# QY-H00/attention-interpolation-diffusion

Hardware: AMD Instinct MI355X
Metric: interpolation-frames/sec (50-step) (higher is better)
Workload: dtype bf16

## Files before the change

attention-interpolation-diffusion_amd/csrc/aid_attn_pp.hip:

```cpp
#include <type_traits>

#include "aid_common.hpp"
#include "aid_kernels.hpp"

namespace aid {

namespace {

constexpr int PKT = 64;
constexpr int PTILE = 8192;
constexpr int PSTAGE = 2 * PTILE;
constexpr int PNS = 8;

struct AttnPPParams {
    AidAttnArgs a;
    int32_t nqb;
    int32_t multi;
    int32_t persist;
    int32_t hv_lo, hv_hi, hv_units;
    float   c2;
#ifdef AID_ABLATIONS
    int32_t abl;
#endif
};
// ... 16 lines not shown
    one[0] = (_Float16)1.0f; one[1] = (_Float16)1.0f;
    return __builtin_amdgcn_fdot2(__builtin_bit_cast(h2, w), one, acc, false);
}

template <typename V>
__device__ __forceinline__ V ld_uniform(const V* ptr, int i) {
    return reinterpret_cast<const __attribute__((address_space(4))) V*>(reinterpret_cast<uintptr_t>(ptr))[i];
}

#ifdef AID_ABLATIONS
#define PP_LDU(ptr, i) ((p.abl & 512) ? (ptr)[i] : ld_uniform(ptr, i))
#else
#define PP_LDU(ptr, i) ld_uniform(ptr, i)
#endif

template <int N>
__device__ __forceinline__ void wait_vm() {
    asm volatile("s_waitcnt vmcnt(%0)" ::"n"(N) : "memory");
}
__device__ __forceinline__ void slot_barrier() {
    __builtin_amdgcn_sched_barrier(0);
    __builtin_amdgcn_s_barrier();
    __builtin_amdgcn_sched_barrier(0);
}

template <typename T, int MODE>
__global__ __launch_bounds__(512) void aid_attn_pp_kernel(const AttnPPParams p) {
    typedef typename Vec<T>::v8 T8;
    typedef typename Vec<T>::v4 T4;
    constexpr int D = 64;
    constexpr float XTH = std::is_same<T, f16>::value ? 15.0f : 60.0f;
    constexpr bool SUMM = std::is_same<T, bf16>::value;
    constexpr float XB = SUMM ? XTH - 1.f : 0.f;
    typedef short s16x4 __attribute__((ext_vector_type(4)));
    extern __shared__ __attribute__((aligned(16))) char smem[];

#ifdef AID_ABLATIONS
    long long tl[6];
    tl[0] = clock64();
#endif
    const AidAttnArgs& a = p.a;
    const int tid = threadIdx.x, lane = tid & 63;
    const int wave = __builtin_amdgcn_readfirstlane(tid >> 6);
    const int grp = wave >> 2;
    const int l31 = lane & 31, hi = lane >> 5;

    const int nt = a.l / PKT;
    const int n_items = p.nqb * a.n_frames * a.heads;
    const int n_heavy = a.n_frames - a.n_plain;
    const bool hf = p.multi && a.n_plain > 0 && n_heavy > 0;
    const int xcd = blockIdx.x & 7, wx = blockIdx.x >> 3, WX = gridDim.x >> 3;
    const int nhf = p.hv_hi - p.hv_lo;
    int pb = 0, npx = 0;
    if (p.persist) {
        const int np = a.heads * p.nqb, q = np >> 3, r = np & 7;
        pb = xcd < r ? xcd * (q + 1) : r * (q + 1) + (xcd - r) * q;
        npx = q + (xcd < r ? 1 : 0);
    }
    int hc = 0, hr = 0, c1 = 0, p2 = 0, nlx = 0;
    if (p.persist) {
        const int nhx = npx * nhf;
        nlx = npx * (a.n_frames - nhf);
        const int hq = nhx / WX;
        hr = nhx % WX;
        hc = hq + (wx < hr ? 1 : 0);
        const int ndef = hr > 0 ? WX - hr : 0;
        p2 = min(nlx, p.hv_units * ndef);
        c1 = (hr > 0 && wx >= hr) ? max(min(p.hv_units * (wx - hr + 1), p2) - p.hv_units * (wx - hr), 0) : 0;
    }
    struct Item { int h, fr, qb; bool ok; };
    auto item_at = [&](int j) __attribute__((always_inline)) -> Item {
        const Item none = {0, 0, 0, false};
        if (!p.persist) {
            if (j != 0) return none;
            const int lid = hf ? heavy_first((int)blockIdx.x, n_items, n_heavy * p.nqb, a.n_frames * p.nqb) : xcd_remap((int)blockIdx.x, n_items);
            if (lid >= n_items) return none;
            return Item{lid / (p.nqb * a.n_frames), (lid / p.nqb) % a.n_frames, lid % p.nqb, true};
        }
// ... 52 lines not shown
        }
        const int kh = N_h * D * 2, vh = N_h * D * a.ldvt * 2;
        N_ks0 = seg0 * (int)a.k_fs * 2 + kh;  N_ks1 = seg1 * (int)a.k_fs * 2 + kh;  N_ks2 = row_e * (int)a.k_fs * 2 + kh;
        N_vs0 = seg0 * (int)a.vt_fs * 2 + vh; N_vs1 = seg1 * (int)a.vt_fs * 2 + vh; N_vs2 = row_e * (int)a.vt_fs * 2 + vh;
    };
    int fr, h, q0, nseg, ks0, ks1, ks2, vs0, vs1, vs2, t2mask, park_at, swap_at, NT;
    float w_b, w_e;
    auto adopt = [&]() __attribute__((always_inline)) {
        fr = N_fr; h = N_h; q0 = N_q0; nseg = N_nseg; ks0 = N_ks0; ks1 = N_ks1; ks2 = N_ks2; vs0 = N_vs0; vs1 = N_vs1; vs2 = N_vs2;
        t2mask = N_t2; park_at = N_park; swap_at = N_swap; w_b = N_wb; w_e = N_we;
        NT = nseg * nt;
    };
    {
        const Item first = item_at(0);
        if (!first.ok) return;
        plan(first);
    }
    if (N_skip) return;
    adopt();

    T8 qf[4];
    auto scale_q = [&]() __attribute__((always_inline)) {
        if (!a.q_prescaled) {
#pragma unroll
            for (int ks = 0; ks < 4; ++ks) {
                f32x8 t = up8<T>(qf[ks]);
#pragma unroll
                for (int e = 0; e < 8; ++e) t[e] *= p.c2;
                qf[ks] = cvt8<T>(t);
            }
        }
    };
    {
        const int qr = min(q0 + l31, a.s - 1);
        const T* qrow = reinterpret_cast<const T*>(a.q) + (int64_t)fr * a.q_fs + (int64_t)qr * a.ldq + h * D;
#pragma unroll
        for (int ks = 0; ks < 4; ++ks) qf[ks] = *reinterpret_cast<const T8*>(qrow + ks * 16 + hi * 8);
        scale_q();
    }

    const Rsrc rk = __builtin_amdgcn_make_buffer_rsrc(const_cast<void*>(a.k), 0, 0x7fffffff, 0x00020000);
    const Rsrc rv = __builtin_amdgcn_make_buffer_rsrc(const_cast<void*>(a.vt), 0, 0x7fffffff, 0x00020000);
    const Rsrc rk2 = __builtin_amdgcn_make_buffer_rsrc(const_cast<void*>(a.k2), 0, 0x7fffffff, 0x00020000);
    const Rsrc rv2 = __builtin_amdgcn_make_buffer_rsrc(const_cast<void*>(a.vt2), 0, 0x7fffffff, 0x00020000);
    const Rsrc rq = __builtin_amdgcn_make_buffer_rsrc(const_cast<void*>(a.q), 0, 0x7fffffff, 0x00020000);
    char* const qlds = smem + 2 * PNS * PTILE + wave * 4096;
    auto dma_q_next = [&]() __attribute__((always_inline)) {
        const int qr = min(N_q0 + l31, a.s - 1);
        const int vo = qr * (a.ldq * 2) + hi * 16;
        const int so = (int)(((int64_t)N_fr * a.q_fs + N_h * D) * 2);
#pragma unroll
        for (int ks = 0; ks < 4; ++ks)
            __builtin_amdgcn_raw_ptr_buffer_load_lds(rq, (__attribute__((address_space(3))) void*)(qlds + ks * 1024), 16, vo, so + ks * 32, 0, 0);
    };
    const int prow = 8 * wave + (lane >> 3);
    const int pch = (lane & 7) ^ ((prow >> 1) & 7);
    const int kvo = prow * (a.ldk * 2) + pch * 16;
    const int vvo = prow * (a.ldvt * 2) + pch * 16;
    int dk = ks0, dv = vs0, dleft = nt, dseg = 0;
    bool d2 = (t2mask & 1) != 0;
    const int kstep = PKT * a.ldk * 2;
    auto dma_next = [&](int st) __attribute__((always_inline)) {
        char* dst = smem + st * PTILE + wave * 1024;
        if (MODE == AID_MODE_INNER && d2) {
            __builtin_amdgcn_raw_ptr_buffer_load_lds(rk2, (__attribute__((address_space(3))) void*)dst, 16, kvo, dk, 0, 0);
            __builtin_amdgcn_raw_ptr_buffer_load_lds(rv2, (__attribute__((address_space(3))) void*)(dst + PNS * PTILE), 16, vvo, dv, 0, 0);
        } else {
            __builtin_amdgcn_raw_ptr_buffer_load_lds(rk, (__attribute__((address_space(3))) void*)dst, 16, kvo, dk, 0, 0);
            __builtin_amdgcn_raw_ptr_buffer_load_lds(rv, (__attribute__((address_space(3))) void*)(dst + PNS * PTILE), 16, vvo, dv, 0, 0);
        }
        dk += kstep;
        dv += PKT * 2;
        if (__builtin_expect(--dleft == 0, 0)) {
            ++dseg;
            dleft = nt;
            if (dseg < nseg) {
                dk = ks1 + (dseg >= 2 ? ks2 - ks1 : 0);
                dv = vs1 + (dseg >= 2 ? vs2 - vs1 : 0);
                d2 = ((t2mask >> dseg) & 1) != 0;
            } else {
                dk = N_ks0;
                dv = N_vs0;
                d2 = (N_t2 & 1) != 0;
            }
        }
    };
    bool has_next = false;

    const int krow = (l31 & 0x13) | ((l31 & 4) << 1) | ((l31 & 8) >> 1);
    const int kx = hi ^ ((krow >> 1) & 7), vx = hi ^ ((l31 >> 1) & 7);
    const int koff = krow * 128, voff = PNS * PTILE + l31 * 128;
    int kad[4], vad[4];
#pragma unroll
    for (int ks = 0; ks < 4; ++ks) {
        kad[ks] = koff + (((2 * ks) ^ kx) << 4);
        vad[ks] = voff + (((2 * ks) ^ vx) << 4);
    }

    float m = 0.f;
    bool fresh = true;
    f32x16 o[2], sc[2];
    float lsum = 0.f;
    f32x4 lacc = {0.f, 0.f, 0.f, 0.f};
    s16x4 ones4;
#pragma unroll
    for (int i = 0; i < 4; ++i) ones4[i] = 0x3f80;
    asm volatile("" : "+v"(ones4));
    auto get_l = [&]() __attribute__((always_inline)) -> float { return SUMM ? lacc[0] : lsum; };
    auto set_l = [&](float x) __attribute__((always_inline)) {
        if (SUMM) { lacc[0] = x; lacc[1] = x; lacc[2] = x; lacc[3] = x; } else lsum = x;
    };
    T8 pf[4];
    f32x16 cneg;
    f32x16 po[2];
    float pl = 0.f, pm = 0.f;
#pragma unroll
    for (int r = 0; r < 16; ++r) { o[0][r] = 0.f; o[1][r] = 0.f; cneg[r] = 0.f; }
    if (MODE == AID_MODE_OUTER) {
#pragma unroll
        for (int r = 0; r < 16; ++r) { po[0][r] = 0.f; po[1][r] = 0.f; }
    }
    asm volatile("" : "+v"(cneg));
#pragma unroll
    for (int i = 0; i < 4; ++i) pf[i] = zero8<T>();

#ifdef AID_ABLATIONS
    long long tmark = clock64();
    float tacc[4] = {0.f, 0.f, 0.f, 0.f};
    auto stamp = [&](int which) __attribute__((always_inline)) {
        if (p.abl & 16) {
            __builtin_amdgcn_sched_barrier(0);
            const long long now = clock64();
            tacc[which] += (float)(now - tmark);
            tmark = now;
            __builtin_amdgcn_sched_barrier(0);
        }
    };
#define PP_STAMP(i) stamp(i)
    long long bt0 = 0;
    uint32_t bt[11];
    for (int i = 0; i < 11; ++i) bt[i] = 0;
    int64_t boff = -1;
    bool barm = false;
    auto bstamp = [&](int which) __attribute__((always_inline)) {
        if (barm) {
            __builtin_amdgcn_sched_barrier(0);
            const long long now = clock64();
            if (which == 0) bt0 = now;
            bt[which] = (uint32_t)(now - bt0);
            __builtin_amdgcn_sched_barrier(0);
        }
    };
#define PP_BSTAMP(i) bstamp(i)
#else
#define PP_STAMP(i)
#define PP_BSTAMP(i) do {} while (0)
#endif

    auto tie = [&]() __attribute__((always_inline)) {
        asm volatile("" : "+v"(sc[0]), "+v"(sc[1]));
        asm volatile("" : "+v"(o[0]), "+v"(o[1]));
        if (SUMM) asm volatile("" : "+v"(lacc));
    };
    auto settle = [&]() __attribute__((always_inline)) {
        tie();
        asm volatile("s_nop 15\n\ts_nop 3" ::: "memory");
        tie();
    };
    T8 kf[4][2], vf[4][2];
    auto lds_k = [&](int st, int ks, int b) __attribute__((always_inline)) {
        return *reinterpret_cast<const T8*>(smem + kad[ks] + (st * PTILE + b * 4096));
    };
    auto lds_v = [&](int st, int kk, int d) __attribute__((always_inline)) {
        return *reinterpret_cast<const T8*>(smem + vad[kk] + (st * PTILE + d * 4096));
    };
    auto pin = []() __attribute__((always_inline)) { __builtin_amdgcn_sched_barrier(0); };

    auto mslot = [&](int sv, int sk) __attribute__((always_inline)) {
#ifdef AID_ABLATIONS
        if (p.abl & 4) {
            asm volatile("" : "+v"(sc[0]), "+v"(sc[1]));
            return;
        }
#endif
        pin();
#pragma unroll
        for (int i = 0; i < 8; ++i) {
            const int ks = i >> 1, b = i & 1;
#ifdef AID_ABLATIONS
            if (!((p.abl & 64) && b))
#endif
            vf[ks][b] = lds_v(sv, ks, b);
            pin();
            sc[b] = mfma32(kf[ks][b], qf[ks], ks ? sc[b] : cneg);
            pin();
        }
#pragma unroll
        for (int i = 0; i < 8; ++i) {
            const int kk = i >> 1, w = i & 1;
            o[w] = mfma32(vf[kk][w], pf[kk], o[w]);
            pin();
            if constexpr (SUMM) {
                const u32x4 w4 = __builtin_bit_cast(u32x4, pf[kk]);
                u32x2 h2;
                h2[0] = w4[2 * w]; h2[1] = w4[2 * w + 1];
                lacc = __builtin_amdgcn_mfma_f32_4x4x4bf16_1k(ones4, __builtin_bit_cast(s16x4, h2), lacc, 0, 0, 0);
                pin();
            }
#ifdef AID_ABLATIONS
            if (!((p.abl & 64) && w))
#endif
            kf[kk][w] = lds_k(sk, kk, w);
            pin();
        }
    };

    constexpr int LEAD = 6;
    auto vslot = [&](int t, bool first) __attribute__((always_inline)) {
#ifdef AID_ABLATIONS
        if (p.abl & 1) {
            if (!(p.abl & 2)) dma_next((t + LEAD) & (PNS - 1));
            fresh = false;
            wait_vm<6>();
            return;
        }
        if (!(p.abl & 2))
#endif
        dma_next((t + LEAD) & (PNS - 1));
        auto exp_tile = [&]() __attribute__((always_inline)) -> float {
            float t0 = 0.f, t1 = 0.f;
#pragma unroll
            for (int b = 0; b < 2; ++b)
#pragma unroll
                for (int u = 0; u < 2; ++u) {
                    f32x8 pv;
#pragma unroll
                    for (int e = 0; e < 8; ++e) pv[e] = __builtin_amdgcn_exp2f(sc[b][8 * u + e]);
                    pf[2 * b + u] = cvt8<T>(pv);
                    const u32x4 w4 = __builtin_bit_cast(u32x4, pf[2 * b + u]);
                    t0 = dot2_ones<T>(w4[0], t0); t1 = dot2_ones<T>(w4[1], t1);
                    t0 = dot2_ones<T>(w4[2], t0); t1 = dot2_ones<T>(w4[3], t1);
                }
            return t0 + t1;
        };
        auto exp_tile_or = [&]() __attribute__((always_inline)) -> uint32_t {
            uint32_t acc = 0;
#pragma unroll
            for (int b = 0; b < 2; ++b)
#pragma unroll
                for (int u = 0; u < 2; ++u) {
                    f32x8 pv;
#pragma unroll
                    for (int e = 0; e < 8; ++e) pv[e] = __builtin_amdgcn_exp2f(sc[b][8 * u + e]);
                    pf[2 * b + u] = cvt8<T>(pv);
                    const u32x4 w4 = __builtin_bit_cast(u32x4, pf[2 * b + u]);
                    acc = (b == 0 && u == 0) ? (w4[0] | w4[1] | w4[2]) | w4[3] : (acc | w4[0] | w4[1]) | (w4[2] | w4[3]);
                }
            return acc;
        };
        auto row_max = [&]() __attribute__((always_inline)) -> float {
            float xm = fmaxf(sc[0][0], sc[0][1]);
#ifdef AID_ABLATIONS
            if (!(p.abl & 8))
#endif
#pragma unroll
            for (int i = 1; i < 16; ++i) xm = fmaxf(fmaxf(xm, sc[i >> 3][(2 * i) & 15]), sc[i >> 3][(2 * i + 1) & 15]);
            return xm;
        };
        auto raise = [&](float xm) __attribute__((always_inline)) {
            settle();
            const float rowmax = max_halves(xm) + XB;
            const float shift = fresh ? rowmax : fmaxf(rowmax, 0.f);
            const float alpha = __builtin_amdgcn_exp2f(-shift);
            m += shift;
#pragma unroll
            for (int r = 0; r < 16; ++r) cneg[r] = -m;
            asm volatile("" : "+v"(cneg));
#pragma unroll
            for (int r = 0; r < 16; ++r) { o[0][r] *= alpha; o[1][r] *= alpha; }
            if (SUMM) lacc *= alpha; else lsum *= alpha;
#pragma unroll
            for (int b = 0; b < 2; ++b)
#pragma unroll
                for (int r = 0; r < 16; ++r) sc[b][r] -= shift;
            fresh = false;
        };
        const bool fr = first && fresh;
        if constexpr (SUMM) {
            const uint32_t orw = fr ? 0u : exp_tile_or();
            if (__builtin_expect(fr || __any((orw & 0x40004000u) != 0u), 0)) {
                raise(row_max());
                exp_tile_or();
            }
        } else {
            float ts = fr ? 0.f : exp_tile();
            if (__builtin_expect(fr || __any(ts > __builtin_amdgcn_exp2f(XTH)), 0)) {
                raise(row_max());
                ts = exp_tile();
            }
            lsum += ts;
        }
        wait_vm<6>();
    };

    auto park = [&]() __attribute__((always_inline)) {
        settle();
#pragma unroll
        for (int r = 0; r < 16; ++r) { po[0][r] = o[0][r]; po[1][r] = o[1][r]; }
        pl = get_l();
        pm = m;
    };
    auto swap_sides = [&]() __attribute__((always_inline)) {
        settle();
        const float lown = get_l();
        const float lrow = lown + other_half(lown);
        const float wb = w_b / lrow;
#pragma unroll
        for (int d = 0; d < 2; ++d)
#pragma unroll
            for (int r = 0; r < 16; ++r) {
                const float rb = o[d][r] * wb;
                o[d][r] = po[d][r];
                po[d][r] = rb;
            }
        set_l(pl);
        const float back = m - pm;
        m = pm;
#pragma unroll
        for (int r = 0; r < 16; ++r) cneg[r] = -m;
        asm volatile("" : "+v"(cneg));
#pragma unroll
        for (int b = 0; b < 2; ++b)
#pragma unroll
            for (int r = 0; r < 16; ++r) sc[b][r] += back;
        if (park_at < 0) fresh = true;
    };

    auto finish = [&]() __attribute__((always_inline)) {
        settle();
#ifdef AID_ABLATIONS
        if (p.abl & (16 | 32)) {
            if (lane == 0 && q0 < a.s) {
                float* dbg = reinterpret_cast<float*>(reinterpret_cast<T*>(a.out) + (int64_t)fr * a.o_fs + (int64_t)q0 * a.ldo + h * D);
                if (p.abl & 16) for (int i = 0; i < 4; ++i) dbg[i] = tacc[i] / (float)NT;
                else { tl[4] = clock64(); for (int i = 1; i < 5; ++i) dbg[i - 1] = (float)(tl[i] - tl[0]); }
            }
            for (int i = 0; i < 4; ++i) tacc[i] = 0.f;
            tmark = clock64();
            return;
        }
#endif
        const float lown = get_l();
        const float inv = w_e / (lown + other_half(lown));
        if (q0 >= a.s) return;
        const float osc = a.out_scale * (a.frame_scale ? PP_LDU(a.frame_scale, fr) : 1.f);
        if (MODE == AID_MODE_OUTER) {
            const int q = q0 + l31;
            if (q < a.s) {
                T* orow = reinterpret_cast<T*>(a.out) + (int64_t)fr * a.o_fs + (int64_t)q * a.ldo + h * D;
#pragma unroll
                for (int d = 0; d < 2; ++d)
#pragma unroll
                    for (int g = 0; g < 4; ++g) {
                        const int dv_ = 32 * d + 8 * g + 4 * hi;
                        f32x4 v;
#pragma unroll
                        for (int e = 0; e < 4; ++e) v[e] = (o[d][4 * g + e] * inv + po[d][4 * g + e]) * osc;
                        if (a.accumulate) v += up4<T>(*reinterpret_cast<const T4*>(orow + dv_));
                        *reinterpret_cast<T4*>(orow + dv_) = cvt4<T>(v);
                    }
            }
        } else {
            char* const st = qlds;
            const int wsw = (l31 >> 1) & 7;
#pragma unroll
            for (int d = 0; d < 2; ++d)
#pragma unroll
                for (int g = 0; g < 4; ++g) {
                    f32x4 v;
#pragma unroll
                    for (int e = 0; e < 4; ++e) v[e] = o[d][4 * g + e] * inv * osc;
                    *reinterpret_cast<T4*>(st + l31 * 128 + (((4 * d + g) ^ wsw) << 4) + 8 * hi) = cvt4<T>(v);
                }
            const Rsrc ro = __builtin_amdgcn_make_buffer_rsrc(a.out, 0, 0x7fffffff, 0x00020000);
            const int so = (int)(((int64_t)fr * a.o_fs + h * D) * 2);
            const int rr = lane >> 3, cc = lane & 7;
#pragma unroll
            for (int i = 0; i < 4; ++i) {
                const int row = rr + 8 * i;
                T8 v = *reinterpret_cast<const T8*>(st + row * 128 + ((cc ^ ((row >> 1) & 7)) << 4));
                const int q = q0 + row;
                const int vo = (min(q, a.s - 1) * a.ldo + cc * 8) * 2;
                if (a.accumulate) v = cvt8<T>(up8<T>(v) + up8<T>(__builtin_bit_cast(T8, __builtin_amdgcn_raw_buffer_load_b128(ro, vo, so, 0))));
                if (q < a.s) __builtin_amdgcn_raw_buffer_store_b128(__builtin_bit_cast(u32x4, v), ro, vo, so, 0);
            }
        }
    };

#pragma unroll
    for (int t = 0; t < LEAD; ++t)
        dma_next(t);
#ifdef AID_ABLATIONS
    if (p.abl & 32) { tl[1] = clock64(); asm volatile("" :: "v"(qf[0]), "v"(qf[3])); }
#endif
    wait_vm<6>();
#ifdef AID_ABLATIONS
    if (p.abl & 32) tl[2] = clock64();
#endif
    slot_barrier();
    if (grp == 1) slot_barrier();
#pragma unroll
    for (int i = 0; i < 8; ++i) kf[i >> 1][i & 1] = lds_k(0, i >> 1, i & 1);
    f32x16 zacc;
#pragma unroll
    for (int r = 0; r < 16; ++r) zacc[r] = 0.f;
#ifdef AID_ABLATIONS
    if (!(p.abl & 4))
#endif
    {
#pragma unroll
        for (int i = 0; i < 8; ++i) sc[i & 1] = mfma32(kf[i >> 1][i & 1], qf[i >> 1], (i >> 1) ? sc[i & 1] : zacc);
        pin();
#pragma unroll
        for (int i = 0; i < 8; ++i) kf[i >> 1][i & 1] = lds_k(1, i >> 1, i & 1);
    }
    settle();
    slot_barrier();
#ifdef AID_ABLATIONS
    if (p.abl & 32) tl[3] = clock64();
#endif
    const bool defer = p.persist && grp == 1;
#pragma nounroll
    for (int j = 0;; ++j) {
        const Item nxt = item_at(j + 1);
        has_next = nxt.ok;
        if (has_next) {
            plan(nxt);
            dma_q_next();
        }
        if (defer && j > 0) slot_barrier();
        PP_BSTAMP(2);
#pragma nounroll
        for (int sgi = 0; sgi < (MODE == AID_MODE_PLAIN ? 1 : nseg); ++sgi) {
            if (MODE == AID_MODE_OUTER) {
                if (sgi == park_at) park();
                if (sgi == swap_at) swap_sides();
            }
            const int t_end = (sgi + 1) * nt;
            for (int t8 = sgi * nt; t8 < t_end; t8 += 8) {
#pragma unroll
                for (int i = 0; i < 8; ++i) {
                    const int t = t8 + i;
                    if (t >= t_end) break;
                    PP_STAMP(3);
                    vslot(t, i == 0);
                    if (i == 7 && __builtin_expect(has_next && t == NT - 1, 0)) {
#pragma unroll
                        for (int ks = 0; ks < 4; ++ks) qf[ks] = *reinterpret_cast<const T8*>(qlds + ks * 1024 + lane * 16);
                        scale_q();
                        m = 0.f;
#pragma unroll
                        for (int r = 0; r < 16; ++r) cneg[r] = 0.f;
                        asm volatile("" : "+v"(cneg));
                    }
                    PP_STAMP(0);
                    if (i < 4) PP_BSTAMP(3 + 2 * i);
                    slot_barrier();
                    PP_STAMP(1);
                    if (i < 4) PP_BSTAMP(4 + 2 * i);
#ifdef AID_ABLATIONS
                    if (i == 3 && barm) {
                        barm = false;
                        if (q0 < a.s) boff = (int64_t)fr * a.o_fs + (int64_t)q0 * a.ldo + h * D;
                    }
#endif
                    mslot(i, (i + 2) & 7);
                    tie();
                    PP_STAMP(2);
                    if (!(i == 7 && defer && t == NT - 1)) slot_barrier();
                }
            }
        }
#ifdef AID_ABLATIONS
        barm = (p.abl & 256) && j == 1 && has_next;
#endif
        PP_BSTAMP(0);
        finish();
        PP_BSTAMP(1);
        if (!has_next) {
            if (defer) slot_barrier();
            break;
        }
        fresh = true;
        set_l(0.f);
        pl = 0.f;
        pm = 0.f;
#pragma unroll
        for (int r = 0; r < 16; ++r) { o[0][r] = 0.f; o[1][r] = 0.f; }
        if (MODE == AID_MODE_OUTER) {
#pragma unroll
            for (int r = 0; r < 16; ++r) { po[0][r] = 0.f; po[1][r] = 0.f; }
        }
        adopt();
        dseg = 0;
    }
    wait_vm<0>();
#ifdef AID_ABLATIONS
    if ((p.abl & 256) && boff >= 0 && lane == 0) {
        uint32_t* dbg = reinterpret_cast<uint32_t*>(reinterpret_cast<T*>(a.out) + boff);
        dbg[0] = 0x50504254u; dbg[1] = 0x4c494e45u;
        for (int i = 0; i < 11; ++i) dbg[2 + i] = bt[i];
    }
#endif
    if (grp == 0) slot_barrier();
}

}

bool attn_pp_supported(const AidAttnArgs& a) {
    const int64_t lim = 1ll << 31;
    const int64_t kb = (int64_t)a.n_kv * a.k_fs * 2, vb = (int64_t)a.n_kv * a.vt_fs * 2;
    const int64_t k2b = a.mode == AID_MODE_INNER ? (int64_t)a.n_frames * a.k_fs * 2 : 0;
    const int64_t v2b = a.mode == AID_MODE_INNER ? (int64_t)a.n_frames * a.vt_fs * 2 : 0;
    const int64_t qb = (int64_t)a.n_frames * a.q_fs * 2, ob = (int64_t)a.n_frames * a.o_fs * 2;
    const uintptr_t al = reinterpret_cast<uintptr_t>(a.k) | reinterpret_cast<uintptr_t>(a.vt) | reinterpret_cast<uintptr_t>(a.k2) |
                         reinterpret_cast<uintptr_t>(a.vt2) | reinterpret_cast<uintptr_t>(a.out);
    const uintptr_t o0 = reinterpret_cast<uintptr_t>(a.out), o1 = o0 + (uintptr_t)ob;
    for (const void* rec : {(const void*)a.coef, (const void*)a.frame_scale, (const void*)a.kv_map}) {
        const uintptr_t r0 = reinterpret_cast<uintptr_t>(rec);
        if (rec && r0 < o1 && o0 < r0 + 4 * (uintptr_t)a.n_frames) return false;
    }
    return a.d == 64 && a.l % PKT == 0 && a.l >= 2 * PKT && a.ldk % 8 == 0 && a.ldvt % 8 == 0 && a.k_fs % 8 == 0 && a.vt_fs % 8 == 0 &&
           (al & 15) == 0 && kb < lim && vb < lim && k2b < lim && v2b < lim && qb < lim && ob < lim && a.ldo % 8 == 0 && a.o_fs % 8 == 0;
}

// ... 45 lines not shown
```

attention-interpolation-diffusion_amd/csrc/aid_common.hpp:

```cpp
#pragma once
#include <hip/hip_runtime.h>
#include <stdint.h>

namespace aid {

typedef _Float16 f16;
typedef __bf16   bf16;

template <typename T> struct Vec;
template <> struct Vec<f16> {
    typedef f16 v2 __attribute__((ext_vector_type(2)));
    typedef f16 v4 __attribute__((ext_vector_type(4)));
    typedef f16 v8 __attribute__((ext_vector_type(8)));
};
template <> struct Vec<bf16> {
    typedef bf16 v2 __attribute__((ext_vector_type(2)));
    typedef bf16 v4 __attribute__((ext_vector_type(4)));
    typedef bf16 v8 __attribute__((ext_vector_type(8)));
};

typedef float f32x2  __attribute__((ext_vector_type(2)));
typedef float f32x4  __attribute__((ext_vector_type(4)));
typedef float f32x8  __attribute__((ext_vector_type(8)));
typedef float f32x16 __attribute__((ext_vector_type(16)));
typedef uint32_t u32x4 __attribute__((ext_vector_type(4)));
typedef uint32_t u32x2 __attribute__((ext_vector_type(2)));

__device__ __forceinline__ f32x16 mfma32(const Vec<f16>::v8& a, const Vec<f16>::v8& b, const f32x16& c) {
    return __builtin_amdgcn_mfma_f32_32x32x16_f16(a, b, c, 0, 0, 0);
}
__device__ __forceinline__ f32x16 mfma32(const Vec<bf16>::v8& a, const Vec<bf16>::v8& b, const f32x16& c) {
    return __builtin_amdgcn_mfma_f32_32x32x16_bf16(a, b, c, 0, 0, 0);
}

template <typename T>
__device__ __forceinline__ typename Vec<T>::v8 zero8() {
    typename Vec<T>::v8 z;
#pragma unroll
    for (int i = 0; i < 8; ++i) z[i] = (T)0.0f;
    return z;
}

template <typename T>
__device__ __forceinline__ typename Vec<T>::v8 cvt8(const f32x8& x) {
    return __builtin_convertvector(x, typename Vec<T>::v8);
}
template <typename T>
__device__ __forceinline__ f32x8 up8(const typename Vec<T>::v8& x) {
    return __builtin_convertvector(x, f32x8);
}
template <typename T>
__device__ __forceinline__ typename Vec<T>::v4 cvt4(const f32x4& x) {
    return __builtin_convertvector(x, typename Vec<T>::v4);
}
template <typename T>
__device__ __forceinline__ f32x4 up4(const typename Vec<T>::v4& x) {
    return __builtin_convertvector(x, f32x4);
}

__device__ __forceinline__ float other_half(float x) {
    const uint32_t u = __float_as_uint(x);
    auto r = __builtin_amdgcn_permlane32_swap(u, u, false, false);
    return (threadIdx.x & 32) ? __uint_as_float(r[0]) : __uint_as_float(r[1]);
}
__device__ __forceinline__ float max_halves(float x) {
    const uint32_t u = __float_as_uint(x);
    auto r = __builtin_amdgcn_permlane32_swap(u, u, false, false);
    return fmaxf(__uint_as_float(r[0]), __uint_as_float(r[1]));
}
__device__ __forceinline__ float sum_halves(float x) {
    const uint32_t u = __float_as_uint(x);
    auto r = __builtin_amdgcn_permlane32_swap(u, u, false, false);
    return __uint_as_float(r[0]) + __uint_as_float(r[1]);
}

__device__ __forceinline__ int xcd_remap(int bid, int nblocks) {
    constexpr int NX = 8;
    const int q = nblocks / NX, r = nblocks % NX;
    const int x = bid % NX, j = bid / NX;
    const int base = (x < r) ? x * (q + 1) : r * (q + 1) + (x - r) * q;
    return base + j;
}

__device__ __forceinline__ int heavy_first(int bid, int nblocks, int na, int per) {
    constexpr int NX = 8;
    const int q = nblocks / NX, r = nblocks % NX;
    const int x = bid % NX, j = bid / NX;
    const int base = (x < r) ? x * (q + 1) : r * (q + 1) + (x - r) * q;
    const int end = base + q + (x < r ? 1 : 0);
    const int nb = per - na;
    const int a0 = (base / per) * na + min(base % per, na);
    const int a1 = (end / per) * na + min(end % per, na);
    if (j < a1 - a0) {
        const int t = a0 + j;
        return (t / na) * per + t % na;
    }
    const int t = (base - a0) + (j - (a1 - a0));
    return (t / nb) * per + na + t % nb;
}


template <typename V>
struct PerDevice {
    static constexpr int MAXD = 64;
    V v[MAXD] = {};
    V* slot() {
// ... 17 lines not shown
```

attention-interpolation-diffusion_amd/csrc/aid_gemm.hip:

```cpp
#include "aid_common.hpp"
#include "aid_kernels.hpp"

#include <stdlib.h>
#include <string.h>

#include <type_traits>

namespace aid {

struct TileCoord {
    int p, batch, m0, n0;
};

template <int NB, int MB>
__device__ __forceinline__ void mfma_fence(f32x16 (&acc)[NB][MB]) {
#pragma unroll
    for (int i = 0; i < NB; ++i)
#pragma unroll
        for (int j = 0; j < MB; ++j) asm volatile("" : "+v"(acc[i][j]));
    asm volatile("s_nop 15\n\ts_nop 3" ::: "memory");
#pragma unroll
    for (int i = 0; i < NB; ++i)
#pragma unroll
        for (int j = 0; j < MB; ++j) asm volatile("" : "+v"(acc[i][j]));
// ... 832 lines not shown

    __device__ __forceinline__ void mac(int kb, int ke) {
        const int nk = ke - kb;
        issue_first<0>(kb, nk);
        if (nk >= 2) wait_vmcnt<2 * (E - 3)>();
        else         wait_vmcnt<0>();
        slot();
        if (wr == 1) slot();
        T8 fa[2][4], fb[2][4];
        for (int kt = 0; kt < nk; ++kt) {
            const char* st = smem + (kt & 1) * STG;
            read_b(fb, st);
            read_a(fa, st, 0);
            retire<0>(kt, nk);
            slot();
            half<0>(fb, fa, kt, kb, nk);
            slot();
            read_a(fa, st, 1);
            retire<1>(kt, nk);
            slot();
            half<1>(fb, fa, kt, kb, nk);
            slot();
        }
        if (wr == 0) slot();
        wait_vmcnt<0>();
        __syncthreads();
    }
};

constexpr int PP_SMALL_NS = 4;
static_assert(Engine<bf16, 128, 128, 64, PP_SMALL_NS, 2, 4>::SMEM <= PingPong<bf16>::SMEM, "small tiles use the big tile's LDS");


__device__ __forceinline__ f32x4 mfma16(const Vec<f16>::v8& a, const Vec<f16>::v8& b, const f32x4& c) {
    return __builtin_amdgcn_mfma_f32_16x16x32_f16(a, b, c, 0, 0, 0);
}
__device__ __forceinline__ f32x4 mfma16(const Vec<bf16>::v8& a, const Vec<bf16>::v8& b, const f32x4& c) {
    return __builtin_amdgcn_mfma_f32_16x16x32_bf16(a, b, c, 0, 0, 0);
}

template <typename T>
struct PingPongX : PingPong<T> {
    typedef PingPong<T> PP;
    typedef typename Vec<T>::v8 T8;
    typedef typename Vec<T>::v4 T4;
    static constexpr int BMX = 288, XR = 32;
    static constexpr int HALF = PP::HALF;
    static constexpr int STGX = 4 * HALF + XR * 128;
    static constexpr int CLD = 256 + 8;
    static constexpr size_t LNS = (size_t)(BMX + 256) * 2 * sizeof(float);
    static constexpr size_t SMEMX = (size_t)BMX * CLD * 2 + LNS > (size_t)2 * STGX ? (size_t)BMX * CLD * 2 + LNS : (size_t)2 * STGX;
    static_assert(SMEMX <= 160 * 1024, "one workgroup per CU");
    using PP::smem; using PP::tid; using PP::lane; using PP::wave; using PP::wm; using PP::wn; using PP::wr;
    using PP::l31; using PP::hi; using PP::aoff; using PP::boff; using PP::ax; using PP::bx; using PP::acc;
    using PP::ra; using PP::rb; using PP::avo; using PP::bvo;
    f32x4 c[2][4][2][2], cx[2][2];
    int l15, kg, a16, b16, x16, cxr, xvo;

    __device__ __forceinline__ void init(char* smem_) {
        PP::init(smem_);
        l15 = lane & 15;
        kg = lane >> 4;
        a16 = (wr * 64 + l15) * 128;
        b16 = 2 * HALF + ((wave & 3) * 32 + l15) * 128;
        x16 = 4 * HALF + l15 * 128;
        cxr = kg ^ PP::swz(l15);
    }
    __device__ __forceinline__ void set_tile(const GemmDesc& P, const T* A, const T* B, int m0, int n0) {
        PP::set_tile(P, A, B, m0, n0);
        const int lrow = 8 * (wave & 3) + (lane >> 3);
        const int c = (lane & 7) ^ PP::swz(lrow);
        xvo = min(256 + lrow, P.m - 1 - m0) * (P.lda * 2) + c * 16;
// ... 911 lines not shown
```

attention-interpolation-diffusion_amd/csrc/aid_gemm_rs.hip:

```cpp
#include "aid_common.hpp"
#include "aid_kernels.hpp"

#include <string.h>

namespace aid {

constexpr int RS_MAXP = 3;
constexpr int RS_NSTG = 3;
constexpr int RS_BIASN = 1280;

struct RsProblem {
    const void* b;
    void*       c;
    const void* bias;
    const void* residual;
    int32_t     n, ldc, trans_rows;
    float       scale;
    int64_t     stride_c;
};

struct RsParams {
    const void* a;
    int32_t     m, n_problems, n_slices, nsplit;
    RsProblem   p[RS_MAXP];
    int32_t     slice_start[RS_MAXP + 1];
};

template <int N>
__device__ __forceinline__ void rs_wait_vm() {
    asm volatile("s_waitcnt vmcnt(%0)" ::"n"(N) : "memory");
}

__device__ __forceinline__ f32x4 mfma16(const Vec<f16>::v8& a, const Vec<f16>::v8& b, const f32x4& c) {
    return __builtin_amdgcn_mfma_f32_16x16x32_f16(a, b, c, 0, 0, 0);
}
__device__ __forceinline__ f32x4 mfma16(const Vec<bf16>::v8& a, const Vec<bf16>::v8& b, const f32x4& c) {
    return __builtin_amdgcn_mfma_f32_16x16x32_bf16(a, b, c, 0, 0, 0);
}

struct RsSrc {
    __amdgpu_buffer_rsrc_t rw;
    int so;
};
template <typename T, int K, int TAG>
__device__ __forceinline__ RsSrc rs_src(const RsParams& p, int s) {
    int pi = 0;
#pragma unroll
    for (int i = 1; i < RS_MAXP; ++i)
        if (i < p.n_problems && s >= p.slice_start[i]) pi = i;
    RsSrc r;
    r.rw = __builtin_amdgcn_make_buffer_rsrc(const_cast<void*>(p.p[pi].b), 0, 0x7fffffff, 0x00020000);
    r.so = (s - p.slice_start[pi]) * (32 * K * 2);
    return r;
}
template <typename T, int TAG>
__device__ __forceinline__ void rs_piece(const RsSrc& src, char* dst, int voff) {
    __builtin_amdgcn_raw_ptr_buffer_load_lds(src.rw, (__attribute__((address_space(3))) void*)dst, 16, voff, src.so, 0, 0);
}

template <typename T, int KT, bool TRANS, int PF>
__device__ __forceinline__ void rs_mac(const char* st, const int (&fr)[2][4], const typename Vec<T>::v8 (&xa)[2][KT], f32x4 (&acc)[2][2],
                                       const char* bias_at, uint32_t (&bq)[4]) {
    typedef typename Vec<T>::v8 T8;
    static_assert(PF >= 1 && PF <= KT, "prefetch window");
    T8 w[PF][2];
#pragma unroll
    for (int j = 0; j < PF; ++j)
#pragma unroll
        for (int a = 0; a < 2; ++a) w[j][a] = *reinterpret_cast<const T8*>(st + fr[a][j & 3] + 256 * (j >> 2));
    if (bias_at) {
        const u32x2 q0 = *reinterpret_cast<const u32x2*>(bias_at), q1 = *reinterpret_cast<const u32x2*>(bias_at + 32);
// ... 330 lines not shown
```

Measured before the change: 4.169.

## Switch ping-pong attention kernel from 32x32 to 16x16 MFMA tiles

Rewrites the attention inner loop to use 16x16x32 MFMA instructions with two 16-row blocks per wave instead of 32x32x16 MFMAs. Q/K/V fragment layouts, LDS addressing, online-softmax state (per-row-block max, sum, alpha) and the epilogue stores are all remapped. The bf16 row-sum now runs on a 16x16 MFMA against a ones vector instead of a 4x4 MFMA, and cross-lane reductions use shuffles over groups of 16 lanes. The aim is better MFMA issue and interleaving granularity with the LDS reads and exp work. In exchange it adds more instructions, extra shuffle reductions, and a risk of layout bugs. The mfma16 helpers move into the common header.

```diff
diff --git a/attention-interpolation-diffusion_amd/csrc/aid_attn_pp.hip b/attention-interpolation-diffusion_amd/csrc/aid_attn_pp.hip
--- a/attention-interpolation-diffusion_amd/csrc/aid_attn_pp.hip
+++ b/attention-interpolation-diffusion_amd/csrc/aid_attn_pp.hip
@@ -72,7 +72,6 @@
     constexpr float XTH = std::is_same<T, f16>::value ? 15.0f : 60.0f;
     constexpr bool SUMM = std::is_same<T, bf16>::value;
     constexpr float XB = SUMM ? XTH - 1.f : 0.f;
-    typedef short s16x4 __attribute__((ext_vector_type(4)));
     extern __shared__ __attribute__((aligned(16))) char smem[];
 
 #ifdef AID_ABLATIONS
@@ -83,7 +82,7 @@
     const int tid = threadIdx.x, lane = tid & 63;
     const int wave = __builtin_amdgcn_readfirstlane(tid >> 6);
     const int grp = wave >> 2;
-    const int l31 = lane & 31, hi = lane >> 5;
+    const int l15 = lane & 15, lg = lane >> 4;
 
     const int nt = a.l / PKT;
     const int n_items = p.nqb * a.n_frames * a.heads;
@@ -202,10 +201,13 @@
         }
     };
     {
-        const int qr = min(q0 + l31, a.s - 1);
-        const T* qrow = reinterpret_cast<const T*>(a.q) + (int64_t)fr * a.q_fs + (int64_t)qr * a.ldq + h * D;
-#pragma unroll
-        for (int ks = 0; ks < 4; ++ks) qf[ks] = *reinterpret_cast<const T8*>(qrow + ks * 16 + hi * 8);
+#pragma unroll
+        for (int rb = 0; rb < 2; ++rb) {
+            const int qr = min(q0 + 16 * rb + l15, a.s - 1);
+            const T* qrow = reinterpret_cast<const T*>(a.q) + (int64_t)fr * a.q_fs + (int64_t)qr * a.ldq + h * D;
+#pragma unroll
+            for (int ks = 0; ks < 2; ++ks) qf[2 * rb + ks] = *reinterpret_cast<const T8*>(qrow + ks * 32 + lg * 8);
+        }
         scale_q();
     }
 
@@ -216,12 +218,15 @@
     const Rsrc rq = __builtin_amdgcn_make_buffer_rsrc(const_cast<void*>(a.q), 0, 0x7fffffff, 0x00020000);
     char* const qlds = smem + 2 * PNS * PTILE + wave * 4096;
     auto dma_q_next = [&]() __attribute__((always_inline)) {
-        const int qr = min(N_q0 + l31, a.s - 1);
-        const int vo = qr * (a.ldq * 2) + hi * 16;
         const int so = (int)(((int64_t)N_fr * a.q_fs + N_h * D) * 2);
 #pragma unroll
-        for (int ks = 0; ks < 4; ++ks)
-            __builtin_amdgcn_raw_ptr_buffer_load_lds(rq, (__attribute__((address_space(3))) void*)(qlds + ks * 1024), 16, vo, so + ks * 32, 0, 0);
+        for (int rb = 0; rb < 2; ++rb) {
+            const int qr = min(N_q0 + 16 * rb + l15, a.s - 1);
+            const int vo = qr * (a.ldq * 2) + lg * 16;
+#pragma unroll
+            for (int ks = 0; ks < 2; ++ks)
+                __builtin_amdgcn_raw_ptr_buffer_load_lds(rq, (__attribute__((address_space(3))) void*)(qlds + (2 * rb + ks) * 1024), 16, vo, so + ks * 64, 0, 0);
+        }
     };
     const int prow = 8 * wave + (lane >> 3);
     const int pch = (lane & 7) ^ ((prow >> 1) & 7);
@@ -257,40 +262,46 @@
     };
     bool has_next = false;
 
-    const int krow = (l31 & 0x13) | ((l31 & 4) << 1) | ((l31 & 8) >> 1);
-    const int kx = hi ^ ((krow >> 1) & 7), vx = hi ^ ((l31 >> 1) & 7);
-    const int koff = krow * 128, voff = PNS * PTILE + l31 * 128;
-    int kad[4], vad[4];
-#pragma unroll
-    for (int ks = 0; ks < 4; ++ks) {
-        kad[ks] = koff + (((2 * ks) ^ kx) << 4);
-        vad[ks] = voff + (((2 * ks) ^ vx) << 4);
-    }
-
-    float m = 0.f;
+    int kad[4], vad[2];
+#pragma unroll
+    for (int ks = 0; ks < 2; ++ks) {
+#pragma unroll
+        for (int b = 0; b < 2; ++b) {
+            const int krow = 8 * (l15 >> 2) + 4 * ((l15 >> 1) & 1) + 2 * b + (l15 & 1);
+            kad[2 * ks + b] = krow * 128 + (((4 * ks + lg) ^ ((krow >> 1) & 7)) << 4);
+        }
+        vad[ks] = PNS * PTILE + l15 * 128 + (((4 * ks + lg) ^ ((l15 >> 1) & 7)) << 4);
+    }
+
+    float m[2] = {0.f, 0.f};
     bool fresh = true;
-    f32x16 o[2], sc[2];
-    float lsum = 0.f;
-    f32x4 lacc = {0.f, 0.f, 0.f, 0.f};
-    s16x4 ones4;
-#pragma unroll
-    for (int i = 0; i < 4; ++i) ones4[i] = 0x3f80;
-    asm volatile("" : "+v"(ones4));
-    auto get_l = [&]() __attribute__((always_inline)) -> float { return SUMM ? lacc[0] : lsum; };
-    auto set_l = [&](float x) __attribute__((always_inline)) {
-        if (SUMM) { lacc[0] = x; lacc[1] = x; lacc[2] = x; lacc[3] = x; } else lsum = x;
+    f32x4 o[8], sc[8];
+    float lsum[2] = {0.f, 0.f};
+    f32x4 lrs[2];
+    T8 ones8;
+#pragma unroll
+    for (int i = 0; i < 8; ++i) ones8[i] = (T)1.0f;
+    asm volatile("" : "+v"(ones8));
+    auto get_l = [&](int rb) __attribute__((always_inline)) -> float { return SUMM ? lrs[rb][0] : lsum[rb]; };
+    auto row_l = [&](int rb) __attribute__((always_inline)) -> float { return SUMM ? lrs[rb][0] : sum_groups4(lsum[rb]); };
+    auto set_l = [&](int rb, float x) __attribute__((always_inline)) {
+        if (SUMM) { lrs[rb][0] = x; lrs[rb][1] = x; lrs[rb][2] = x; lrs[rb][3] = x; } else lsum[rb] = x;
     };
     T8 pf[4];
-    f32x16 cneg;
-    f32x16 po[2];
-    float pl = 0.f, pm = 0.f;
-#pragma unroll
-    for (int r = 0; r < 16; ++r) { o[0][r] = 0.f; o[1][r] = 0.f; cneg[r] = 0.f; }
-    if (MODE == AID_MODE_OUTER) {
-#pragma unroll
-        for (int r = 0; r < 16; ++r) { po[0][r] = 0.f; po[1][r] = 0.f; }
-    }
-    asm volatile("" : "+v"(cneg));
+    f32x4 cneg[2];
+    f32x4 po[8];
+    float pl[2] = {0.f, 0.f}, pm[2] = {0.f, 0.f};
+#pragma unroll
+    for (int i = 0; i < 8; ++i)
+#pragma unroll
+        for (int r = 0; r < 4; ++r) { o[i][r] = 0.f; if (MODE == AID_MODE_OUTER) po[i][r] = 0.f; }
+#pragma unroll
+    for (int rb = 0; rb < 2; ++rb) {
+        set_l(rb, 0.f);
+#pragma unroll
+        for (int r = 0; r < 4; ++r) cneg[rb][r] = 0.f;
+    }
+    asm volatile("" : "+v"(cneg[0]), "+v"(cneg[1]));
 #pragma unroll
     for (int i = 0; i < 4; ++i) pf[i] = zero8<T>();
 
@@ -328,60 +339,67 @@
 #endif
 
     auto tie = [&]() __attribute__((always_inline)) {
-        asm volatile("" : "+v"(sc[0]), "+v"(sc[1]));
-        asm volatile("" : "+v"(o[0]), "+v"(o[1]));
-        if (SUMM) asm volatile("" : "+v"(lacc));
+#pragma unroll
+        for (int i = 0; i < 8; ++i) asm volatile("" : "+v"(sc[i]), "+v"(o[i]));
+        if (SUMM) asm volatile("" : "+v"(lrs[0]), "+v"(lrs[1]));
     };
     auto settle = [&]() __attribute__((always_inline)) {
         tie();
         asm volatile("s_nop 15\n\ts_nop 3" ::: "memory");
         tie();
     };
-    T8 kf[4][2], vf[4][2];
-    auto lds_k = [&](int st, int ks, int b) __attribute__((always_inline)) {
-        return *reinterpret_cast<const T8*>(smem + kad[ks] + (st * PTILE + b * 4096));
-    };
-    auto lds_v = [&](int st, int kk, int d) __attribute__((always_inline)) {
-        return *reinterpret_cast<const T8*>(smem + vad[kk] + (st * PTILE + d * 4096));
+    T8 kf[2][4], vf[2][4];
+    auto lds_k = [&](int st, int ks, int kb) __attribute__((always_inline)) {
+        return *reinterpret_cast<const T8*>(smem + kad[2 * ks + (kb & 1)] + (st * PTILE + (kb >> 1) * 4096));
+    };
+    auto lds_v = [&](int st, int ks, int cb) __attribute__((always_inline)) {
+        return *reinterpret_cast<const T8*>(smem + vad[ks] + (st * PTILE + cb * 2048));
     };
     auto pin = []() __attribute__((always_inline)) { __builtin_amdgcn_sched_barrier(0); };
 
     auto mslot = [&](int sv, int sk) __attribute__((always_inline)) {
 #ifdef AID_ABLATIONS
         if (p.abl & 4) {
-            asm volatile("" : "+v"(sc[0]), "+v"(sc[1]));
+#pragma unroll
+            for (int i = 0; i < 8; ++i) asm volatile("" : "+v"(sc[i]));
             return;
         }
 #endif
         pin();
 #pragma unroll
-        for (int i = 0; i < 8; ++i) {
-            const int ks = i >> 1, b = i & 1;
-#ifdef AID_ABLATIONS
-            if (!((p.abl & 64) && b))
-#endif
-            vf[ks][b] = lds_v(sv, ks, b);
+        for (int i = 0; i < 16; ++i) {
+            const int ks = i >> 3, kb = (i >> 1) & 3, rb = i & 1;
+            if (!(i & 1)) {
+                const int n = i >> 1;
+#ifdef AID_ABLATIONS
+                if (!((p.abl & 64) && (n & 1)))
+#endif
+                vf[n >> 2][n & 3] = lds_v(sv, n >> 2, n & 3);
+                pin();
+            }
+            sc[2 * kb + rb] = mfma16(kf[ks][kb], qf[2 * rb + ks], ks ? sc[2 * kb + rb] : cneg[rb]);
             pin();
-            sc[b] = mfma32(kf[ks][b], qf[ks], ks ? sc[b] : cneg);
-            pin();
-        }
-#pragma unroll
-        for (int i = 0; i < 8; ++i) {
-            const int kk = i >> 1, w = i & 1;
-            o[w] = mfma32(vf[kk][w], pf[kk], o[w]);
+        }
+#pragma unroll
+        for (int i = 0; i < 16; ++i) {
+            const int ks = i >> 3, cb = (i >> 1) & 3, rb = i & 1;
+            o[2 * cb + rb] = mfma16(vf[ks][cb], pf[2 * rb + ks], o[2 * cb + rb]);
             pin();
             if constexpr (SUMM) {
-                const u32x4 w4 = __builtin_bit_cast(u32x4, pf[kk]);
-                u32x2 h2;
-                h2[0] = w4[2 * w]; h2[1] = w4[2 * w + 1];
-                lacc = __builtin_amdgcn_mfma_f32_4x4x4bf16_1k(ones4, __builtin_bit_cast(s16x4, h2), lacc, 0, 0, 0);
+                if ((i & 3) == 3) {
+                    const int j = i >> 2, rs = j & 1, kq = j >> 1;
+                    lrs[rs] = mfma16(ones8, pf[2 * rs + kq], lrs[rs]);
+                    pin();
+                }
+            }
+            if (i & 1) {
+                const int n = i >> 1;
+#ifdef AID_ABLATIONS
+                if (!((p.abl & 64) && (n & 1)))
+#endif
+                kf[n >> 2][n & 3] = lds_k(sk, n >> 2, n & 3);
                 pin();
             }
-#ifdef AID_ABLATIONS
-            if (!((p.abl & 64) && w))
-#endif
-            kf[kk][w] = lds_k(sk, kk, w);
-            pin();
         }
     };
 
@@ -397,78 +415,80 @@
         if (!(p.abl & 2))
 #endif
         dma_next((t + LEAD) & (PNS - 1));
-        auto exp_tile = [&]() __attribute__((always_inline)) -> float {
-            float t0 = 0.f, t1 = 0.f;
-#pragma unroll
-            for (int b = 0; b < 2; ++b)
-#pragma unroll
-                for (int u = 0; u < 2; ++u) {
-                    f32x8 pv;
-#pragma unroll
-                    for (int e = 0; e < 8; ++e) pv[e] = __builtin_amdgcn_exp2f(sc[b][8 * u + e]);
-                    pf[2 * b + u] = cvt8<T>(pv);
-                    const u32x4 w4 = __builtin_bit_cast(u32x4, pf[2 * b + u]);
-                    t0 = dot2_ones<T>(w4[0], t0); t1 = dot2_ones<T>(w4[1], t1);
-                    t0 = dot2_ones<T>(w4[2], t0); t1 = dot2_ones<T>(w4[3], t1);
+        auto exp_frag = [&](int rb, int ks) __attribute__((always_inline)) -> u32x4 {
+            f32x8 pv;
+#pragma unroll
+            for (int e = 0; e < 8; ++e) pv[e] = __builtin_amdgcn_exp2f(sc[2 * (2 * ks + ((e >> 1) & 1)) + rb][(e & 1) + 2 * (e >> 2)]);
+            pf[2 * rb + ks] = cvt8<T>(pv);
+            return __builtin_bit_cast(u32x4, pf[2 * rb + ks]);
+        };
+        auto exp_tile = [&](float& s0, float& s1) __attribute__((always_inline)) {
+            float t[2] = {0.f, 0.f};
+#pragma unroll
+            for (int ks = 0; ks < 2; ++ks)
+#pragma unroll
+                for (int rb = 0; rb < 2; ++rb) {
+                    const u32x4 w4 = exp_frag(rb, ks);
+#pragma unroll
+                    for (int e = 0; e < 4; ++e) t[rb] = dot2_ones<T>(w4[e], t[rb]);
                 }
-            return t0 + t1;
+            s0 = t[0]; s1 = t[1];
         };
         auto exp_tile_or = [&]() __attribute__((always_inline)) -> uint32_t {
             uint32_t acc = 0;
 #pragma unroll
-            for (int b = 0; b < 2; ++b)
-#pragma unroll
-                for (int u = 0; u < 2; ++u) {
-                    f32x8 pv;
-#pragma unroll
-                    for (int e = 0; e < 8; ++e) pv[e] = __builtin_amdgcn_exp2f(sc[b][8 * u + e]);
-                    pf[2 * b + u] = cvt8<T>(pv);
-                    const u32x4 w4 = __builtin_bit_cast(u32x4, pf[2 * b + u]);
-                    acc = (b == 0 && u == 0) ? (w4[0] | w4[1] | w4[2]) | w4[3] : (acc | w4[0] | w4[1]) | (w4[2] | w4[3]);
+            for (int ks = 0; ks < 2; ++ks)
+#pragma unroll
+                for (int rb = 0; rb < 2; ++rb) {
+                    const u32x4 w4 = exp_frag(rb, ks);
+                    acc = (ks == 0 && rb == 0) ? (w4[0] | w4[1] | w4[2]) | w4[3] : (acc | w4[0] | w4[1]) | (w4[2] | w4[3]);
                 }
             return acc;
         };
-        auto row_max = [&]() __attribute__((always_inline)) -> float {
-            float xm = fmaxf(sc[0][0], sc[0][1]);
+        auto row_max = [&](int rb) __attribute__((always_inline)) -> float {
+            float xm = fmaxf(sc[rb][0], sc[rb][1]);
 #ifdef AID_ABLATIONS
             if (!(p.abl & 8))
 #endif
 #pragma unroll
-            for (int i = 1; i < 16; ++i) xm = fmaxf(fmaxf(xm, sc[i >> 3][(2 * i) & 15]), sc[i >> 3][(2 * i + 1) & 15]);
+            for (int i = 1; i < 8; ++i) xm = fmaxf(fmaxf(xm, sc[2 * (i >> 1) + rb][(2 * i) & 3]), sc[2 * (i >> 1) + rb][(2 * i + 1) & 3]);
             return xm;
         };
-        auto raise = [&](float xm) __attribute__((always_inline)) {
+        auto raise = [&]() __attribute__((always_inline)) {
             settle();
-            const float rowmax = max_halves(xm) + XB;
-            const float shift = fresh ? rowmax : fmaxf(rowmax, 0.f);
-            const float alpha = __builtin_amdgcn_exp2f(-shift);
-            m += shift;
-#pragma unroll
-            for (int r = 0; r < 16; ++r) cneg[r] = -m;
-            asm volatile("" : "+v"(cneg));
-#pragma unroll
-            for (int r = 0; r < 16; ++r) { o[0][r] *= alpha; o[1][r] *= alpha; }
-            if (SUMM) lacc *= alpha; else lsum *= alpha;
-#pragma unroll
-            for (int b = 0; b < 2; ++b)
-#pragma unroll
-                for (int r = 0; r < 16; ++r) sc[b][r] -= shift;
+#pragma unroll
+            for (int rb = 0; rb < 2; ++rb) {
+                const float rowmax = max_groups4(row_max(rb)) + XB;
+                const float shift = fresh ? rowmax : fmaxf(rowmax, 0.f);
+                const float alpha = __builtin_amdgcn_exp2f(-shift);
+                m[rb] += shift;
+#pragma unroll
+                for (int r = 0; r < 4; ++r) cneg[rb][r] = -m[rb];
+#pragma unroll
+                for (int cb = 0; cb < 4; ++cb) o[2 * cb + rb] *= alpha;
+                if (SUMM) lrs[rb] *= alpha; else lsum[rb] *= alpha;
+#pragma unroll
+                for (int kb = 0; kb < 4; ++kb) sc[2 * kb + rb] -= shift;
+            }
+            asm volatile("" : "+v"(cneg[0]), "+v"(cneg[1]));
             fresh = false;
         };
         const bool fr = first && fresh;
         if constexpr (SUMM) {
             const uint32_t orw = fr ? 0u : exp_tile_or();
             if (__builtin_expect(fr || __any((orw & 0x40004000u) != 0u), 0)) {
-                raise(row_max());
+                raise();
                 exp_tile_or();
             }
         } else {
-            float ts = fr ? 0.f : exp_tile();
-            if (__builtin_expect(fr || __any(ts > __builtin_amdgcn_exp2f(XTH)), 0)) {
-                raise(row_max());
-                ts = exp_tile();
-            }
-            lsum += ts;
+            float ts0 = 0.f, ts1 = 0.f;
+            if (!fr) exp_tile(ts0, ts1);
+            if (__builtin_expect(fr || __any(fmaxf(ts0, ts1) > __builtin_amdgcn_exp2f(XTH)), 0)) {
+                raise();
+                exp_tile(ts0, ts1);
+            }
+            lsum[0] += ts0;
+            lsum[1] += ts1;
         }
         wait_vm<6>();
     };
@@ -476,33 +496,30 @@
     auto park = [&]() __attribute__((always_inline)) {
         settle();
 #pragma unroll
-        for (int r = 0; r < 16; ++r) { po[0][r] = o[0][r]; po[1][r] = o[1][r]; }
-        pl = get_l();
-        pm = m;
+        for (int i = 0; i < 8; ++i) po[i] = o[i];
+#pragma unroll
+        for (int rb = 0; rb < 2; ++rb) { pl[rb] = get_l(rb); pm[rb] = m[rb]; }
     };
     auto swap_sides = [&]() __attribute__((always_inline)) {
         settle();
-        const float lown = get_l();
-        const float lrow = lown + other_half(lown);
-        const float wb = w_b / lrow;
-#pragma unroll
-        for (int d = 0; d < 2; ++d)
-#pragma unroll
-            for (int r = 0; r < 16; ++r) {
-                const float rb = o[d][r] * wb;
-                o[d][r] = po[d][r];
-                po[d][r] = rb;
-            }
-        set_l(pl);
-        const float back = m - pm;
-        m = pm;
-#pragma unroll
-        for (int r = 0; r < 16; ++r) cneg[r] = -m;
-        asm volatile("" : "+v"(cneg));
-#pragma unroll
-        for (int b = 0; b < 2; ++b)
-#pragma unroll
-            for (int r = 0; r < 16; ++r) sc[b][r] += back;
+#pragma unroll
+        for (int rb = 0; rb < 2; ++rb) {
+            const float wb = w_b / row_l(rb);
+#pragma unroll
+            for (int cb = 0; cb < 4; ++cb) {
+                const f32x4 rbk = o[2 * cb + rb] * wb;
+                o[2 * cb + rb] = po[2 * cb + rb];
+                po[2 * cb + rb] = rbk;
+            }
+            set_l(rb, pl[rb]);
+            const float back = m[rb] - pm[rb];
+            m[rb] = pm[rb];
+#pragma unroll
+            for (int r = 0; r < 4; ++r) cneg[rb][r] = -m[rb];
+#pragma unroll
+            for (int kb = 0; kb < 4; ++kb) sc[2 * kb + rb] += back;
+        }
+        asm volatile("" : "+v"(cneg[0]), "+v"(cneg[1]));
         if (park_at < 0) fresh = true;
     };
 
@@ -520,37 +537,35 @@
             return;
         }
 #endif
-        const float lown = get_l();
-        const float inv = w_e / (lown + other_half(lown));
+        float inv[2];
+#pragma unroll
+        for (int rb = 0; rb < 2; ++rb) inv[rb] = w_e / row_l(rb);
         if (q0 >= a.s) return;
         const float osc = a.out_scale * (a.frame_scale ? PP_LDU(a.frame_scale, fr) : 1.f);
         if (MODE == AID_MODE_OUTER) {
-            const int q = q0 + l31;
-            if (q < a.s) {
-                T* orow = reinterpret_cast<T*>(a.out) + (int64_t)fr * a.o_fs + (int64_t)q * a.ldo + h * D;
-#pragma unroll
-                for (int d = 0; d < 2; ++d)
-#pragma unroll
-                    for (int g = 0; g < 4; ++g) {
-                        const int dv_ = 32 * d + 8 * g + 4 * hi;
-                        f32x4 v;
-#pragma unroll
-                        for (int e = 0; e < 4; ++e) v[e] = (o[d][4 * g + e] * inv + po[d][4 * g + e]) * osc;
+#pragma unroll
+            for (int rb = 0; rb < 2; ++rb) {
+                const int q = q0 + 16 * rb + l15;
+                if (q < a.s) {
+                    T* orow = reinterpret_cast<T*>(a.out) + (int64_t)fr * a.o_fs + (int64_t)q * a.ldo + h * D;
+#pragma unroll
+                    for (int cb = 0; cb < 4; ++cb) {
+                        const int dv_ = 16 * cb + 4 * lg;
+                        f32x4 v = (o[2 * cb + rb] * inv[rb] + po[2 * cb + rb]) * osc;
                         if (a.accumulate) v += up4<T>(*reinterpret_cast<const T4*>(orow + dv_));
                         *reinterpret_cast<T4*>(orow + dv_) = cvt4<T>(v);
                     }
+                }
             }
         } else {
             char* const st = qlds;
-            const int wsw = (l31 >> 1) & 7;
-#pragma unroll
-            for (int d = 0; d < 2; ++d)
-#pragma unroll
-                for (int g = 0; g < 4; ++g) {
-                    f32x4 v;
-#pragma unroll
-                    for (int e = 0; e < 4; ++e) v[e] = o[d][4 * g + e] * inv * osc;
-                    *reinterpret_cast<T4*>(st + l31 * 128 + (((4 * d + g) ^ wsw) << 4) + 8 * hi) = cvt4<T>(v);
+            const int wsw = (l15 >> 1) & 7;
+#pragma unroll
+            for (int rb = 0; rb < 2; ++rb)
+#pragma unroll
+                for (int cb = 0; cb < 4; ++cb) {
+                    const f32x4 v = o[2 * cb + rb] * inv[rb] * osc;
+                    *reinterpret_cast<T4*>(st + (16 * rb + l15) * 128 + (((2 * cb + (lg >> 1)) ^ wsw) << 4) + 8 * (lg & 1)) = cvt4<T>(v);
                 }
             const Rsrc ro = __builtin_amdgcn_make_buffer_rsrc(a.out, 0, 0x7fffffff, 0x00020000);
             const int so = (int)(((int64_t)fr * a.o_fs + h * D) * 2);
@@ -580,19 +595,20 @@
     slot_barrier();
     if (grp == 1) slot_barrier();
 #pragma unroll
-    for (int i = 0; i < 8; ++i) kf[i >> 1][i & 1] = lds_k(0, i >> 1, i & 1);
-    f32x16 zacc;
-#pragma unroll
-    for (int r = 0; r < 16; ++r) zacc[r] = 0.f;
+    for (int i = 0; i < 8; ++i) kf[i >> 2][i & 3] = lds_k(0, i >> 2, i & 3);
+    const f32x4 zacc = {0.f, 0.f, 0.f, 0.f};
 #ifdef AID_ABLATIONS
     if (!(p.abl & 4))
 #endif
     {
 #pragma unroll
-        for (int i = 0; i < 8; ++i) sc[i & 1] = mfma32(kf[i >> 1][i & 1], qf[i >> 1], (i >> 1) ? sc[i & 1] : zacc);
+        for (int i = 0; i < 16; ++i) {
+            const int ks = i >> 3, kb = (i >> 1) & 3, rb = i & 1;
+            sc[2 * kb + rb] = mfma16(kf[ks][kb], qf[2 * rb + ks], ks ? sc[2 * kb + rb] : zacc);
+        }
         pin();
 #pragma unroll
-        for (int i = 0; i < 8; ++i) kf[i >> 1][i & 1] = lds_k(1, i >> 1, i & 1);
+        for (int i = 0; i < 8; ++i) kf[i >> 2][i & 3] = lds_k(1, i >> 2, i & 3);
     }
     settle();
     slot_barrier();
@@ -628,10 +644,10 @@
 #pragma unroll
                         for (int ks = 0; ks < 4; ++ks) qf[ks] = *reinterpret_cast<const T8*>(qlds + ks * 1024 + lane * 16);
                         scale_q();
-                        m = 0.f;
-#pragma unroll
-                        for (int r = 0; r < 16; ++r) cneg[r] = 0.f;
-                        asm volatile("" : "+v"(cneg));
+                        m[0] = 0.f; m[1] = 0.f;
+#pragma unroll
+                        for (int r = 0; r < 4; ++r) { cneg[0][r] = 0.f; cneg[1][r] = 0.f; }
+                        asm volatile("" : "+v"(cneg[0]), "+v"(cneg[1]));
                     }
                     PP_STAMP(0);
                     if (i < 4) PP_BSTAMP(3 + 2 * i);
@@ -662,15 +678,12 @@
             break;
         }
         fresh = true;
-        set_l(0.f);
-        pl = 0.f;
-        pm = 0.f;
-#pragma unroll
-        for (int r = 0; r < 16; ++r) { o[0][r] = 0.f; o[1][r] = 0.f; }
-        if (MODE == AID_MODE_OUTER) {
-#pragma unroll
-            for (int r = 0; r < 16; ++r) { po[0][r] = 0.f; po[1][r] = 0.f; }
-        }
+#pragma unroll
+        for (int rb = 0; rb < 2; ++rb) { set_l(rb, 0.f); pl[rb] = 0.f; pm[rb] = 0.f; }
+#pragma unroll
+        for (int i = 0; i < 8; ++i)
+#pragma unroll
+            for (int r = 0; r < 4; ++r) { o[i][r] = 0.f; if (MODE == AID_MODE_OUTER) po[i][r] = 0.f; }
         adopt();
         dseg = 0;
     }
diff --git a/attention-interpolation-diffusion_amd/csrc/aid_common.hpp b/attention-interpolation-diffusion_amd/csrc/aid_common.hpp
--- a/attention-interpolation-diffusion_amd/csrc/aid_common.hpp
+++ b/attention-interpolation-diffusion_amd/csrc/aid_common.hpp
@@ -31,6 +31,13 @@
 }
 __device__ __forceinline__ f32x16 mfma32(const Vec<bf16>::v8& a, const Vec<bf16>::v8& b, const f32x16& c) {
     return __builtin_amdgcn_mfma_f32_32x32x16_bf16(a, b, c, 0, 0, 0);
+}
+
+__device__ __forceinline__ f32x4 mfma16(const Vec<f16>::v8& a, const Vec<f16>::v8& b, const f32x4& c) {
+    return __builtin_amdgcn_mfma_f32_16x16x32_f16(a, b, c, 0, 0, 0);
+}
+__device__ __forceinline__ f32x4 mfma16(const Vec<bf16>::v8& a, const Vec<bf16>::v8& b, const f32x4& c) {
+    return __builtin_amdgcn_mfma_f32_16x16x32_bf16(a, b, c, 0, 0, 0);
 }
 
 template <typename T>
@@ -72,6 +79,15 @@
     const uint32_t u = __float_as_uint(x);
     auto r = __builtin_amdgcn_permlane32_swap(u, u, false, false);
     return __uint_as_float(r[0]) + __uint_as_float(r[1]);
+}
+
+__device__ __forceinline__ float max_groups4(float x) {
+    x = fmaxf(x, __shfl_xor(x, 16));
+    return fmaxf(x, __shfl_xor(x, 32));
+}
+__device__ __forceinline__ float sum_groups4(float x) {
+    x += __shfl_xor(x, 16);
+    return x + __shfl_xor(x, 32);
 }
 
 __device__ __forceinline__ int xcd_remap(int bid, int nblocks) {
diff --git a/attention-interpolation-diffusion_amd/csrc/aid_gemm.hip b/attention-interpolation-diffusion_amd/csrc/aid_gemm.hip
--- a/attention-interpolation-diffusion_amd/csrc/aid_gemm.hip
+++ b/attention-interpolation-diffusion_amd/csrc/aid_gemm.hip
@@ -888,12 +888,6 @@
 static_assert(Engine<bf16, 128, 128, 64, PP_SMALL_NS, 2, 4>::SMEM <= PingPong<bf16>::SMEM, "small tiles use the big tile's LDS");
 
 
-__device__ __forceinline__ f32x4 mfma16(const Vec<f16>::v8& a, const Vec<f16>::v8& b, const f32x4& c) {
-    return __builtin_amdgcn_mfma_f32_16x16x32_f16(a, b, c, 0, 0, 0);
-}
-__device__ __forceinline__ f32x4 mfma16(const Vec<bf16>::v8& a, const Vec<bf16>::v8& b, const f32x4& c) {
-    return __builtin_amdgcn_mfma_f32_16x16x32_bf16(a, b, c, 0, 0, 0);
-}
 
 template <typename T>
 struct PingPongX : PingPong<T> {
diff --git a/attention-interpolation-diffusion_amd/csrc/aid_gemm_rs.hip b/attention-interpolation-diffusion_amd/csrc/aid_gemm_rs.hip
--- a/attention-interpolation-diffusion_amd/csrc/aid_gemm_rs.hip
+++ b/attention-interpolation-diffusion_amd/csrc/aid_gemm_rs.hip
@@ -31,12 +31,6 @@
     asm volatile("s_waitcnt vmcnt(%0)" ::"n"(N) : "memory");
 }
 
-__device__ __forceinline__ f32x4 mfma16(const Vec<f16>::v8& a, const Vec<f16>::v8& b, const f32x4& c) {
-    return __builtin_amdgcn_mfma_f32_16x16x32_f16(a, b, c, 0, 0, 0);
-}
-__device__ __forceinline__ f32x4 mfma16(const Vec<bf16>::v8& a, const Vec<bf16>::v8& b, const f32x4& c) {
-    return __builtin_amdgcn_mfma_f32_16x16x32_bf16(a, b, c, 0, 0, 0);
-}
 
 struct RsSrc {
     __amdgpu_buffer_rsrc_t rw;
```

Result: faster. 4.256 (median of 6 runs) (+2.1%).
